# tsnorri/vcf2multialign

Measured on AMD Instinct MI355X. Metric: aligned A2M Gbases/sec, higher is better.
Workload: dtype u8

## Files before the change

### vcf2multialign_amd/csrc/kernels.hpp

```cpp
#pragma once

#include <hip/hip_runtime.h>
#include <stdint.h>

#ifdef V2M_CHECKED_BUILD
__device__ uint32_t v2m_lds_poison_seed;
#endif

namespace v2m {

typedef uint32_t u32;
typedef uint64_t u64;

constexpr int kWave = 64;
typedef u32 vec4u __attribute__((ext_vector_type(4)));
typedef vec4u vec4u_unaligned8 __attribute__((aligned(8)));

#ifdef V2M_CHECKED_BUILD
__device__ __forceinline__ u32 poison_hash(u32 seed, u32 wg, u32 i)
{
	u32 h = seed ^ (wg * 0x9E3779B1u) ^ (i * 0x85EBCA77u);
	h ^= h >> 15; h *= 0x2C1B3C6Du;
	h ^= h >> 12; h *= 0x297A2D39u;
	h ^= h >> 15;
// ... 808 lines not shown
	u32 const *record_offset;
	u32 const *edge_end;
};

__global__ __launch_bounds__(256) void expand_reference_set_kernel(
	char const *__restrict__ ref, u32 const *__restrict__ ref_pos, u32 const *__restrict__ aln_pos,
	u32 n_nodes, set_tile_tables st, u32 n_tiles, u64 n_chunks, uint4 *__restrict__ out, char gap)
{
	u64 const c = (u64) blockIdx.x * blockDim.x + threadIdx.x;
	if (c >= n_chunks) return;
	u32 lo = 0, hi = n_tiles;
	while (hi - lo > 1) {
		u32 const mid = lo + (hi - lo) / 2;
		if ((u64) st.record_offset[mid] <= c * 16) lo = mid; else hi = mid;
	}
	u64 const p0 = (u64) st.col_begin[lo] + (c * 16 - st.record_offset[lo]);
	out[c] = expand_reference_chunk(ref, ref_pos, aln_pos, n_nodes, st.col_end[lo], p0, gap, (unsigned char) gap);
}


struct row_segments {
	u32 const *seg_offsets;
	u32 const *seg_edge_begin;
	u32 const *seg_copy;
	u64 const *assembled;
	u32 assembled_words;
};

__device__ __forceinline__ u64 load_row_word(
	u64 const *__restrict__ paths, u64 words_per_copy, row_segments const &rs, u32 row, u32 s_begin, u32 s_end, u32 wi)
{
	if (s_end - s_begin == 1) {
		u32 const copy = rs.seg_copy[s_begin];
		return (copy == 0xFFFFFFFFu) ? 0 : paths[(u64) copy * words_per_copy + wi];
	}
	return rs.assembled[(u64) row * rs.assembled_words + wi];
}

__global__ __launch_bounds__(256) void assemble_row_bits_kernel(
	u64 const *__restrict__ paths, u64 words_per_copy, row_segments rs, u64 *__restrict__ assembled, u32 n_words, u32 row_base, u32 word_base)
{
	__shared__ unsigned long long acc[256];
	u32 const row = blockIdx.y + row_base;
	u32 const s_begin = rs.seg_offsets[row], s_end = rs.seg_offsets[row + 1];
	if (s_end - s_begin <= 1) return;
	V2M_POISON_LDS(acc);
	u32 const lane = threadIdx.x & 63, wave = threadIdx.x >> 6;
	u32 const w0 = word_base + (blockIdx.x * 4 + wave) * 64;
	acc[threadIdx.x] = 0;
	__syncthreads();
	if (w0 < n_words) {
		u64 const e_lo = (u64) w0 * 64;
		u64 const e_hi = (u64) (w0 + 64 < n_words ? w0 + 64 : n_words) * 64;
		u32 lo = s_begin, hi = s_end;
		while (hi - lo > 1) {
			u32 const mid = lo + (hi - lo) / 2;
			if (rs.seg_edge_begin[mid] <= e_lo) lo = mid; else hi = mid;
		}
		for (u32 s = lo + lane; s < s_end; s += 64) {
			u64 b = rs.seg_edge_begin[s];
			if (b >= e_hi) break;
			u64 e = (s + 1 < s_end) ? rs.seg_edge_begin[s + 1] : ~0ULL;
			u32 const copy = rs.seg_copy[s];
			if (copy == 0xFFFFFFFFu) continue;
			b = b > e_lo ? b : e_lo;
			e = e < e_hi ? e : e_hi;
			if (b >= e) continue;
			u64 const *const column = paths + (u64) copy * words_per_copy;
			for (u64 wi = b >> 6; wi <= (e - 1) >> 6; ++wi) {
				u64 const base = wi * 64;
				u32 const from = b > base ? (u32) (b - base) : 0;
				u32 const to = e < base + 64 ? (u32) (e - base) : 64;
				u64 const mask = (to >= 64 ? ~0ULL : ((1ULL << to) - 1)) & ~((1ULL << from) - 1);
				u64 const v = column[wi] & mask;
				if (v) atomicOr(&acc[wave * 64 + (u32) (wi - w0)], (unsigned long long) v);
			}
		}
	}
	__syncthreads();
	if (w0 + lane < n_words) assembled[(u64) row * rs.assembled_words + w0 + lane] = acc[threadIdx.x];
}

constexpr int kResolveWordsPerThread = 8;
constexpr u32 kResolveQueueShards = 1024;
constexpr u32 kMaxBackWords = 2048;

__device__ __forceinline__ u64 resolve_word_exact(
	u64 const *__restrict__ paths, u64 words_per_copy, row_segments const &rs, u32 row, u32 s_begin, u32 s_end,
	edge_span const *__restrict__ spans, u64 const *__restrict__ overlappable,
	u32 wi, u64 w, u64 ovl_w, u32 *__restrict__ needs_serial, u32 max_back_words)
{
	u64 const ov = w & ovl_w;
	if (0 == ov) return w;
	int const b0 = __builtin_ctzll(ov);
	u32 sw = wi;
	int sb = 0;
	u64 fixed = ~ovl_w & ((1ULL << b0) - 1);
	if (fixed) {
		sb = 63 - __builtin_clzll(fixed);
	} else {
		u32 steps = 0;
		for (;;) {
			if (0 == sw) { sb = 0; break; }
			--sw;
			if (++steps > max_back_words) { atomicOr(&needs_serial[row], 1u); return w; }
			fixed = ~overlappable[sw];
			if (fixed) { sb = 63 - __builtin_clzll(fixed); break; }
		}
	}
	u64 out = (sw == wi) ? (w & ((1ULL << sb) - 1)) : 0;
	u32 cur = 0;
	for (u32 ww = sw; ww <= wi; ++ww) {
		u64 x = (ww == wi) ? w : load_row_word(paths, words_per_copy, rs, row, s_begin, s_end, ww);
		if (ww == sw) x &= ~((1ULL << sb) - 1);
		while (x) {
			constexpr int kBatch = 8;
			edge_span sp[kBatch];
			int bit[kBatch];
			bool has[kBatch];
#pragma unroll
			for (int k = 0; k < kBatch; ++k) {
				has[k] = 0 != x;
				bit[k] = has[k] ? __builtin_ctzll(x) : 0;
				x &= x - 1;
				sp[k] = spans[ww * 64u + bit[k]];
			}
#pragma unroll
			for (int k = 0; k < kBatch; ++k) {
				if (has[k] && sp[k].src >= cur) {
					cur = sp[k].tgt;
					if (ww == wi) out |= 1ULL << bit[k];
				}
			}
		}
	}
	return out;
}

__global__ __launch_bounds__(256) void resolve_effective_edges_kernel(
	u64 const *__restrict__ paths, u64 words_per_copy, u32 n_edges,
	row_segments rs, edge_span const *__restrict__ spans, u64 const *__restrict__ overlappable,
	u32 const *__restrict__ ovl_rank, u64 const *__restrict__ blocker_masks,
	u64 *__restrict__ eff, u32 n_words, u32 eff_words_per_row, u32 row_base, u32 word_base,
	u32 *__restrict__ queue, u32 *__restrict__ queue_counts , u32 shard_capacity, u32 *__restrict__ needs_serial, u32 max_back_words)
{
	u32 const row = blockIdx.x + row_base;
	u32 const shard = (blockIdx.y * gridDim.x + blockIdx.x) % kResolveQueueShards;
	u32 const s_begin = rs.seg_offsets[row], s_end = rs.seg_offsets[row + 1];
	u64 const tail_mask = (n_edges & 63) ? (1ULL << (n_edges & 63)) - 1 : ~0ULL;
	u64 const *row_words = nullptr;
	if (s_end - s_begin == 1) {
		u32 const copy = rs.seg_copy[s_begin];
		if (copy != 0xFFFFFFFFu) row_words = paths + (u64) copy * words_per_copy;
	} else {
		row_words = rs.assembled + (u64) row * rs.assembled_words;
	}
	u32 const w_first = word_base + blockIdx.y * kResolveWordsPerThread * blockDim.x + threadIdx.x;
	u64 w_all[kResolveWordsPerThread], ovl_all[kResolveWordsPerThread], mask_a[kResolveWordsPerThread], mask_b[kResolveWordsPerThread];
	u32 rank_all[kResolveWordsPerThread];
#pragma unroll
	for (int piece = 0; piece < kResolveWordsPerThread; ++piece) {
		u32 const wi = w_first + piece * blockDim.x;
		u32 const wc = wi < n_words ? wi : n_words - 1;
		w_all[piece] = row_words ? row_words[wc] : 0;
		ovl_all[piece] = overlappable[wc];
		rank_all[piece] = ovl_rank[wc];
		if (wi == (n_edges - 1) >> 6) w_all[piece] &= tail_mask;
	}
#pragma unroll
	for (int piece = 0; piece < kResolveWordsPerThread; ++piece) {
		u64 const ov = w_all[piece] & ovl_all[piece], ov2 = ov & (ov - 1);
		auto const entry = [&](u64 m) {
			return m ? rank_all[piece] + (u32) __builtin_popcountll(ovl_all[piece] & ((1ULL << __builtin_ctzll(m)) - 1)) : 0u;
		};
		mask_a[piece] = blocker_masks[entry(ov)];
		mask_b[piece] = blocker_masks[entry(ov2)];
	}
	int const lane = threadIdx.x & 63;
#pragma unroll
	for (int piece = 0; piece < kResolveWordsPerThread; ++piece) {
		u32 const wi = w_first + piece * blockDim.x;
		bool const in_range = wi < n_words;
		u64 const w = w_all[piece], ov = w & ovl_all[piece], ov2 = ov & (ov - 1);
		bool const hard = in_range && ov && ((w & mask_a[piece]) || (ov2 && ((w & mask_b[piece]) || (ov2 & (ov2 - 1)))));
		if (in_range && !hard) eff[(u64) row * eff_words_per_row + wi] = w;
		u64 const hard_lanes = __ballot(hard);
		if (hard_lanes) {
			u32 base = 0;
			if (0 == lane) base = atomicAdd(&queue_counts[shard], (u32) __builtin_popcountll(hard_lanes));
			base = __shfl(base, 0, kWave);
			if (hard) {
				u32 const slot = base + __builtin_amdgcn_mbcnt_hi((u32) (hard_lanes >> 32), __builtin_amdgcn_mbcnt_lo((u32) hard_lanes, 0));
				if (slot < shard_capacity) queue[(u64) shard * shard_capacity + slot] = (row - row_base) * n_words + wi;
				else eff[(u64) row * eff_words_per_row + wi] = resolve_word_exact(paths, words_per_copy, rs, row, s_begin, s_end, spans, overlappable, wi, w, ovl_all[piece], needs_serial, max_back_words);
			}
		}
	}
}

__global__ __launch_bounds__(256) void resolve_queued_words_kernel(
	u64 const *__restrict__ paths, u64 words_per_copy, u32 n_edges,
	row_segments rs, edge_span const *__restrict__ spans, u64 const *__restrict__ overlappable,
	u64 *__restrict__ eff, u32 n_words, u32 eff_words_per_row, u32 row_base,
	u32 const *__restrict__ queue, u32 const *__restrict__ queue_counts, u32 shard_capacity, u32 *__restrict__ needs_serial, u32 max_back_words)
{
	u32 const shard = blockIdx.x % kResolveQueueShards, part = blockIdx.x / kResolveQueueShards, parts = gridDim.x / kResolveQueueShards;
	u32 const n = queue_counts[shard] < shard_capacity ? queue_counts[shard] : shard_capacity;
	u64 const tail_mask = (n_edges & 63) ? (1ULL << (n_edges & 63)) - 1 : ~0ULL;
	for (u32 i = part * blockDim.x + threadIdx.x; i < n; i += parts * blockDim.x) {
		u32 const entry = queue[(u64) shard * shard_capacity + i];
		u32 const row = row_base + entry / n_words, wi = entry % n_words;
		u32 const s_begin = rs.seg_offsets[row], s_end = rs.seg_offsets[row + 1];
		u64 w = load_row_word(paths, words_per_copy, rs, row, s_begin, s_end, wi);
		if (wi == (n_edges - 1) >> 6) w &= tail_mask;
		eff[(u64) row * eff_words_per_row + wi] = resolve_word_exact(paths, words_per_copy, rs, row, s_begin, s_end, spans, overlappable, wi, w, overlappable[wi], needs_serial, max_back_words);
	}
}


__global__ __launch_bounds__(256) void resolve_rows_serial_kernel(
	u64 const *__restrict__ paths, u64 words_per_copy, u32 n_edges,
	row_segments rs, edge_span const *__restrict__ spans,
	u64 *__restrict__ eff, u64 eff_words_per_row, u32 n_rows, u32 const *__restrict__ needs_serial,
	u32 word_begin , u32 word_end)
{
	int const lane = threadIdx.x & 63;
	u32 const row = blockIdx.x * (blockDim.x >> 6) + (threadIdx.x >> 6);
	if (row >= n_rows) return;
	if (needs_serial && 0 == needs_serial[row]) return;

	u32 const s_begin = rs.seg_offsets[row], s_end = rs.seg_offsets[row + 1];
	u32 const n_words = (n_edges + 63) / 64;
	u64 *const eff_row = eff + (u64) row * eff_words_per_row;
	u32 cur = 0;

	for (u32 base = word_begin; base < word_end; base += 64) {
		u32 const wi = base + lane;
		u64 w = 0;
		if (wi < word_end) {
			w = load_row_word(paths, words_per_copy, rs, row, s_begin, s_end, wi);
			if (wi == n_words - 1 && (n_edges & 63))
				w &= (1ULL << (n_edges & 63)) - 1;
		}

		u32 lane_max = 0;
		for (u64 m = w; m; m &= m - 1) {
			u32 const e = wi * 64u + __builtin_ctzll(m);
			u32 const tgt = spans[e].tgt;
			lane_max = tgt > lane_max ? tgt : lane_max;
		}
		u32 incl = lane_max;
#pragma unroll
		for (int d = 1; d < 64; d <<= 1) {
			u32 const o = __shfl_up(incl, d, kWave);
			if (lane >= d) incl = o > incl ? o : incl;
		}
		u32 excl = __shfl_up(incl, 1, kWave);
		if (lane == 0) excl = 0;
		u32 const chunk_max = __shfl(incl, 63, kWave);

		u32 run = excl > cur ? excl : cur;
		bool uncertain = false;
		for (u64 m = w; m; m &= m - 1) {
			u32 const e = wi * 64u + __builtin_ctzll(m);
			edge_span const sp = spans[e];
			uncertain |= sp.src < run;
			run = sp.tgt > run ? sp.tgt : run;
		}

		u64 out = w;
		if (__any(uncertain)) {
			out = 0;
			u32 c = cur;
			u64 busy = __ballot(w != 0);
			while (busy) {
				int const j = __builtin_ctzll(busy);
				busy &= busy - 1;
				if (lane == j) {
					for (u64 m = w; m; m &= m - 1) {
// ... 1256 lines not shown
```

### vcf2multialign_amd/csrc/v2m_hip.hip

```cpp

#include <hip/hip_runtime.h>

#include <algorithm>
#include <atomic>
#include <chrono>
#include <condition_variable>
#include <cstdarg>
#include <cstdio>
#include <cstdlib>
#include <cstring>
#include <memory>
#include <mutex>
#include <string>
#include <thread>
#include <utility>
#include <vector>

#include <type_traits>

#include "../../include/v2m_hip.h"
#include "kernels.hpp"
#include "founder_kernels.hpp"
#include "bgzf_kernels.hpp"
#include "vcf_kernels.hpp"
// ... 103 lines not shown
struct held_ring_state {
	std::mutex mutex;
	std::condition_variable released;
};

struct v2m_row_hold {
	pinned_buf host;
	hipEvent_t copied{};
	uint64_t outstanding{};
	held_ring_state *ring{};
};


struct word_range { u64 restart, lo, hi, stride; };

struct row_view {
	u64 begin{}, end{};
	u64 max_unaligned{};
	u32 n_tiles{};
	dev_buf d_template, d_template0;
	bool has_template0{};
	dev_buf d_edge_begin, d_cross_offsets, d_cross_edges;
	word_range words{};
	u64 length() const { return end - begin; }
};


struct v2m_ctx {
	int device{};
	u32 n_cus{256};
	hipStream_t stream{};
	hipStream_t copy_stream{};
	std::string err;

	bool profiling{};
	std::vector<event_pair> events[V2M_KERNEL_END];
	std::vector<event_pair> free_events;

	bool has_graph{};
	u64 n_nodes{}, n_edges{}, ref_len{}, aligned_len{}, label_bytes{};
	bool has_nul_byte{};
	std::vector<u32> h_csum;
	std::vector<u32> h_tgt_prefix_max;
	dev_buf d_ref, d_ref_pos, d_aln_pos, d_spans, d_patches, d_labels, d_overlappable;
	dev_buf d_ovl_rank, d_blocker_masks;
	std::vector<u32> h_aln_pos, h_tile_edge_begin, h_cross_offsets, h_cross_edges;
	std::vector<v2m::edge_patch> h_patches;
	std::vector<u64> h_overlappable;

	row_view whole, window;
	bool windowed{};
	row_view &view() { return set_call ? set.view : windowed ? window : whole; }
	row_view const &view() const { return set_call ? set.view : windowed ? window : whole; }

	struct window_set {
		row_view view;
		u64 n_windows{}, pitch{}, mean_tile_bytes{};
		std::vector<u32> lengths;
		dev_buf d_col_begin, d_col_end, d_record_offset, d_edge_end, d_tile_window, d_first_tile, d_slot_offset32;
	} set;
	bool has_set{}, set_call{};
	scratch_buf d_set_tile_offsets, d_set_lengths[2];
	int set_lengths_slot{};

	u64 const *d_paths{};
	dev_buf owned_paths;
	dev_buf d_slice_src;
	u64 path_rows{}, path_cols{};
	u64 path_pitch{};
	dev_buf d_by_edge;
	bool by_edge_valid{};

	struct transpose_pick { u64 rows, cols, src_pitch, dst_pitch; std::string kernel; };
	std::vector<transpose_pick> transpose_choice;

	int store_mode{-1};
	int unaligned_store_mode{-1};
	std::string info;

	pinned_buf h_row_stage[2];
	hipEvent_t ev_row_stage[2]{};
	bool row_stage_in_flight[2]{};
	int row_stage_next{};
	scratch_buf d_resolve_queue, d_resolve_count;
	scratch_buf d_eff, d_row_bits, d_seg_offsets, d_seg_edge_begin, d_seg_copy, d_sums, d_lengths, d_needs_serial, d_tile_counts, d_row_lengths;
	scratch_buf ring[2];
	dev_buf d_ops_ref_before;
	bool has_ops_ref_before{};
	scratch_buf d_ops_info, d_ops_offsets, d_ops_counts, d_ops_base, d_ops_out;
	pinned_buf h_ops_stage, h_ops_out;
	std::vector<v2m_aln_op> ops_row;
	held_ring_state held_state;
	std::vector<std::unique_ptr<v2m_row_hold>> host_slots;
	pinned_buf trials_stage[2];
	scratch_buf d_bgzf_slots, d_bgzf_sizes, d_bgzf_offsets, d_bgzf_table, d_bgzf_dense[2], d_bgzf_in;
	pinned_buf h_bgzf_table[2];
	hipEvent_t ev_compute[2]{};
	scratch_buf d_inflate_in[2], d_inflate_out[2], d_inflate_status[2];
	hipEvent_t ev_inflate_in[2]{};
	dev_buf d_vcf_text[2];
	scratch_buf d_vcf_in, d_vcf_status, d_vcf_tiles, d_vcf_tile_offsets, d_vcf_line_start, d_vcf_lines, d_vcf_gt_off, d_vcf_flags, d_vcf_tmp_begin,
		d_vcf_tmp_columns, d_vcf_totals, d_vcf_heads, d_vcf_columns, d_vcf_layout, d_vcf_wanted;
};


namespace {

int fail(v2m_ctx *ctx, int code, char const *fmt, ...)
{
	char buf[512];
	va_list ap;
	va_start(ap, fmt);
	std::vsnprintf(buf, sizeof(buf), fmt, ap);
	va_end(ap);
	if (ctx) ctx->err = buf; else g_create_error = buf;
	return code;
}

#define V2M_HIP_TRY(ctx, expr)                                                              \
	do {                                                                                    \
		hipError_t const st_ = (expr);                                                      \
		if (hipSuccess != st_) {                                                            \
			int const code_ = (hipErrorOutOfMemory == st_) ? V2M_ERR_OUT_OF_MEMORY : V2M_ERR_HIP; \
			return fail(ctx, code_, "%s failed: %s", #expr, hipGetErrorString(st_));       \
		}                                                                                   \
	} while (0)


struct timed_launch {
	v2m_ctx *ctx;
	int kernel;
	event_pair ev{};
	bool active{};

	timed_launch(v2m_ctx *c, int k) : ctx(c), kernel(k)
	{
		if (!ctx->profiling) return;
		if (!ctx->free_events.empty()) { ev = ctx->free_events.back(); ctx->free_events.pop_back(); }
		else if (hipSuccess != hipEventCreate(&ev.begin) || hipSuccess != hipEventCreate(&ev.end)) return;
		active = (hipSuccess == hipEventRecord(ev.begin, ctx->stream));
	}
	~timed_launch()
	{
		if (!active) return;
		(void) hipEventRecord(ev.end, ctx->stream);
		ctx->events[kernel].push_back(ev);
	}
};


template <typename T>
int upload_vec(v2m_ctx *ctx, dev_buf &dst, std::vector<T> const &src, size_t min_bytes = 16)
{
	size_t const bytes(std::max(src.size() * sizeof(T), min_bytes));
	V2M_HIP_TRY(ctx, dst.ensure(bytes));
	if (!src.empty())
		V2M_HIP_TRY(ctx, hipMemcpyAsync(dst.p, src.data(), src.size() * sizeof(T), hipMemcpyHostToDevice, ctx->stream));
	return V2M_OK;
}


struct scoped_events {
	std::vector<hipEvent_t> ev;
	~scoped_events() { for (auto e : ev) (void) hipEventDestroy(e); }
	hipError_t create(std::size_t n)
	{
		for (std::size_t i(0); i < n; ++i) {
			hipEvent_t e{};
// ... 234 lines not shown
	if (shape == "stream4x64") return launch_transpose_stream<4, 16, 4, 4, 64>(ctx, d_src, SW, DW, SP, DP, d_dst, xcd, order);
#endif
	if (shape == "8x8") return launch_transpose_shape<8, 8>(ctx, d_src, SW, DW, SP, DP, d_dst, xcd, order);
#ifdef V2M_TUNING_BUILD
	if (shape == "4x16") return launch_transpose_shape<4, 16>(ctx, d_src, SW, DW, SP, DP, d_dst, xcd, order);
	if (shape == "16x8") return launch_transpose_shape<16, 8>(ctx, d_src, SW, DW, SP, DP, d_dst, xcd, order);
	if (shape == "16x4") return launch_transpose_shape<16, 4>(ctx, d_src, SW, DW, SP, DP, d_dst, xcd, order);
	if (shape == "4x8") return launch_transpose_shape<4, 8>(ctx, d_src, SW, DW, SP, DP, d_dst, xcd, order);
	if (shape == "8x4") return launch_transpose_shape<8, 4>(ctx, d_src, SW, DW, SP, DP, d_dst, xcd, order);
	if (shape == "8x16") return launch_transpose_shape<8, 16>(ctx, d_src, SW, DW, SP, DP, d_dst, xcd, order);
#endif
	return fail(ctx, V2M_ERR_INVALID_ARGUMENT, "unknown transpose kernel '%s'", shape.c_str());
}

char const *const kTransposeCandidates[] = {"8x8", "stream16", "lines8", "lines16"};

int launch_transpose(v2m_ctx *ctx, u64 const *d_src, u64 n_rows, u64 n_cols, u64 *d_dst, u64 src_pitch = 0, u64 dst_pitch = 0)
{
	u64 const SW(n_rows / 64), DW(n_cols / 64);
	u64 const SP(src_pitch ? src_pitch : SW), DP(dst_pitch ? dst_pitch : DW);
	char const *e(std::getenv("V2M_TRANSPOSE_PANEL"));
	if (e && *e) return launch_transpose_named(ctx, e, d_src, SW, DW, SP, DP, d_dst);
	if (SW * DW * 512 < (u64(32) << 20)) return launch_transpose_named(ctx, "8x8", d_src, SW, DW, SP, DP, d_dst);
	for (auto const &c : ctx->transpose_choice)
		if (c.rows == n_rows && c.cols == n_cols && c.src_pitch == SP && c.dst_pitch == DP) return launch_transpose_named(ctx, c.kernel, d_src, SW, DW, SP, DP, d_dst);

	std::vector<std::string> names;
	if (char const *list = std::getenv("V2M_TRANSPOSE_CANDIDATES")) {
		std::string cur;
		for (char const *p(list); ; ++p) {
			if (';' == *p || 0 == *p) { if (!cur.empty()) names.push_back(cur); cur.clear(); if (0 == *p) break; }
			else cur.push_back(*p);
		}
	}
	if (names.empty()) names.assign(std::begin(kTransposeCandidates), std::end(kTransposeCandidates));

	std::vector<float> best(names.size(), 1e30f);
	{
		scoped_events ev;
		V2M_HIP_TRY(ctx, ev.create(names.size() + 1));
		scoped_profiling_off const quiet(ctx);
		std::vector<char> usable(names.size(), 1);
		for (int rep(0); rep < 3; ++rep) {
			V2M_HIP_TRY(ctx, hipEventRecord(ev[0], ctx->stream));
			for (std::size_t k(0); k < names.size(); ++k) {
				if (usable[k]) {
					int const rc(launch_transpose_named(ctx, names[k], d_src, SW, DW, SP, DP, d_dst));
					if (V2M_ERR_UNSUPPORTED == rc) usable[k] = 0;
					else if (rc) return rc;
				}
				V2M_HIP_TRY(ctx, hipEventRecord(ev[k + 1], ctx->stream));
			}
			V2M_HIP_TRY(ctx, hipStreamSynchronize(ctx->stream));
			for (std::size_t k(0); k < names.size(); ++k) {
				float ms(0);
				V2M_HIP_TRY(ctx, hipEventElapsedTime(&ms, ev[k], ev[k + 1]));
				if (rep && usable[k]) best[k] = std::min(best[k], ms);
			}
		}
		if (std::none_of(usable.begin(), usable.end(), [](char u) { return 0 != u; })) return fail(ctx, V2M_ERR_UNSUPPORTED, "matrix too large for one transpose launch");
		if (std::any_of(usable.begin(), usable.end(), [](char u) { return 0 == u; })) ctx->err.clear();
	}
	std::size_t const pick(std::size_t(std::min_element(best.begin(), best.end()) - best.begin()));
	ctx->transpose_choice.push_back({n_rows, n_cols, SP, DP, names[pick]});
	std::string note("transpose " + std::to_string(n_rows) + "x" + std::to_string(n_cols) + " bits" + ((SP != SW || DP != DW) ? " (column pitches " + std::to_string(SP) + " / " + std::to_string(DP) + " words)" : std::string()) + ": " + names[pick] + " (");
	for (std::size_t k(0); k < names.size(); ++k) {
		char buf[64];
		std::snprintf(buf, sizeof(buf), "%s%s %.3f ms", k ? ", " : "", names[k].c_str(), best[k]);
		note += buf;
	}
	note += ")";
	if (ctx->info.size() > 2000) ctx->info.clear();
	if (!ctx->info.empty()) ctx->info += "; ";
	ctx->info += note;
	return launch_transpose_named(ctx, names[pick], d_src, SW, DW, SP, DP, d_dst);
}


struct prepared_rows {
	u32 *seg_offsets{};
	u32 *seg_edge_begin{};
	u32 *seg_copy{};
	u64 n_rows{}, n_segments{};
	bool any_switching_row{};
};

int prepare_rows(v2m_ctx *ctx, v2m_row_batch const *rows, u64 row_begin, u64 row_end, prepared_rows &out)
{
	u64 const n_rows(row_end - row_begin);
	u64 max_segments(n_rows);
	if (rows->cut_offsets) {
		for (u64 r(row_begin); r < row_end; ++r) {
			if (rows->cut_offsets[r + 1] < rows->cut_offsets[r])
				return fail(ctx, V2M_ERR_INVALID_ARGUMENT, "cut_offsets decrease at row %llu", (unsigned long long) r);
			max_segments += rows->cut_offsets[r + 1] - rows->cut_offsets[r];
		}
	}
	if (max_segments >= 0xFFFFFFFFull)
		return fail(ctx, V2M_ERR_UNSUPPORTED, "row batch has too many cut segments (%llu) for one call", (unsigned long long) max_segments);
	auto const pad([](u64 n) { return (n * sizeof(u32) + 63) & ~u64(63); });
	int const area(ctx->row_stage_next);
	if (ctx->row_stage_in_flight[area]) {
		V2M_HIP_TRY(ctx, hipEventSynchronize(ctx->ev_row_stage[area]));
		ctx->row_stage_in_flight[area] = false;
	}
	V2M_HIP_TRY(ctx, ctx->h_row_stage[area].ensure(pad(n_rows + 1) + 2 * pad(max_segments)));
	char *const base(static_cast<char *>(ctx->h_row_stage[area].p));
	V2M_POISON_HOST(base, pad(n_rows + 1) + 2 * pad(max_segments));
	out.seg_offsets = reinterpret_cast<u32 *>(base);
	out.seg_edge_begin = reinterpret_cast<u32 *>(base + pad(n_rows + 1));
	out.seg_copy = reinterpret_cast<u32 *>(base + pad(n_rows + 1) + pad(max_segments));
	out.n_rows = n_rows;
	out.any_switching_row = false;

	out.seg_offsets[0] = 0;
	for (u64 r(row_begin); r < row_end; ++r) {
		u64 const c_begin(rows->cut_offsets ? rows->cut_offsets[r] : 0), c_end(rows->cut_offsets ? rows->cut_offsets[r + 1] : 0);
		u64 const n_seg(c_begin == c_end ? 1 : (c_end - c_begin) + (0 != rows->cut_nodes[c_begin] ? 1 : 0));
		out.seg_offsets[r - row_begin + 1] = u32(out.seg_offsets[r - row_begin] + n_seg);
		out.any_switching_row = out.any_switching_row || n_seg > 1;
	}
	out.n_segments = out.seg_offsets[n_rows];

	struct row_error { int code{V2M_OK}; std::string text; };
	auto const fill_row([&](u64 r, row_error &err) {
		auto const failed([&](int code, char const *fmt, unsigned long long a, unsigned long long b = 0) {
			char buf[256];
			std::snprintf(buf, sizeof(buf), fmt, a, b);
			err.code = code;
			err.text = buf;
		});
		u64 const c_begin(rows->cut_offsets ? rows->cut_offsets[r] : 0), c_end(rows->cut_offsets ? rows->cut_offsets[r + 1] : 0);
		u32 n(out.seg_offsets[r - row_begin]);
		if (c_begin == c_end) {
			if (!rows->copy_index) return failed(V2M_ERR_INVALID_ARGUMENT, "row %llu has no cuts and rows->copy_index is NULL", r);
			u32 const copy(rows->copy_index[r]);
			if (copy != V2M_PLOIDY_MAX && (!ctx->d_paths || copy >= ctx->path_cols))
				return failed(V2M_ERR_INVALID_ARGUMENT, "row %llu: chromosome copy %llu is outside the path matrix", r, copy);
			out.seg_edge_begin[n] = 0;
			out.seg_copy[n] = copy;
			return;
		}
		u64 prev(0);
		for (u64 k(c_begin); k < c_end; ++k) {
			u64 const node(rows->cut_nodes[k]);
			u32 const copy(rows->cut_copies[k]);
			if (node >= ctx->n_nodes) return failed(V2M_ERR_PRECONDITION, "row %llu: cut node %llu does not exist", r, node);
			if (k > c_begin && node <= prev) return failed(V2M_ERR_PRECONDITION, "row %llu: cut nodes must be strictly increasing", r);
			if (copy != V2M_PLOIDY_MAX && (!ctx->d_paths || copy >= ctx->path_cols))
				return failed(V2M_ERR_INVALID_ARGUMENT, "row %llu: chromosome copy %llu is outside the path matrix", r, copy);
			u32 const first_edge(ctx->h_csum[node]);
			if (node > 0 && ctx->h_tgt_prefix_max[first_edge] > node)
				return failed(V2M_ERR_PRECONDITION, "row %llu: cut node %llu lies inside the span of an ALT edge", r, node);
			if (k == c_begin && node != 0) {
				out.seg_edge_begin[n] = 0;
				out.seg_copy[n] = V2M_PLOIDY_MAX;
				++n;
			}
			out.seg_edge_begin[n] = first_edge;
			out.seg_copy[n] = copy;
			++n;
			prev = node;
		}
	});
	std::vector<row_error> errors(n_rows);
	unsigned const n_threads(out.n_segments >= (u64(1) << 20) ? unsigned(std::min<u64>(n_rows, 8)) : 1u);
	if (n_threads <= 1) {
		for (u64 r(row_begin); r < row_end; ++r) { fill_row(r, errors[r - row_begin]); if (V2M_OK != errors[r - row_begin].code) break; }
	}
	else {
		std::atomic<u64> next(row_begin);
		auto const work([&] { for (u64 r; (r = next.fetch_add(1)) < row_end;) fill_row(r, errors[r - row_begin]); });
		std::vector<std::thread> pool;
		for (unsigned t(1); t < n_threads; ++t) pool.emplace_back(work);
		work();
		for (auto &t : pool) t.join();
	}
	for (auto const &e : errors) if (V2M_OK != e.code) return fail(ctx, e.code, "%s", e.text.c_str());
	return V2M_OK;
}


int forced_store_mode(bool unaligned)
{
	if (unaligned) {
		char const *const e = std::getenv("V2M_UNALIGNED_STORE");
		if (e && 0 == std::strcmp(e, "plain")) return 0;
		if (e && 0 == std::strcmp(e, "nt")) return 1;
		return -1;
	}
	char const *e = std::getenv("V2M_NT_STORES");
	if (!(e && *e)) return -1;
	return std::atoi(e) != 0 ? 1 : 0;
}

u32 rows_per_group_for(u64 n_rows)
{
	char const *e = std::getenv("V2M_ROWS_PER_GROUP");
	int const v((e && *e) ? std::atoi(e) : 0);
	if (v > 0) return u32(std::min(v, 256));
	return u32(std::min<u64>(32, std::max<u64>(1, n_rows)));
}


u32 rows_per_group_for_set(u64 n_rows, u64 mean_tile_bytes)
{
	char const *e = std::getenv("V2M_ROWS_PER_GROUP");
	if (e && *e && std::atoi(e) > 0) return rows_per_group_for(n_rows);
	u64 const by_bytes(32 * u64(v2m::kTileBytes) / std::max<u64>(1, mean_tile_bytes));
	return u32(std::min<u64>(std::max<u64>(1, n_rows), std::min<u64>(256, std::max<u64>(32, by_bytes))));
}


int expand_reference(v2m_ctx *ctx, row_view const &v, dev_buf &dst, char gap)
{
	u64 const n_chunks(u64(v.n_tiles) * v2m::kTileChunks);
	V2M_HIP_TRY(ctx, dst.ensure(n_chunks * 16));
	{
		timed_launch tl(ctx, V2M_KERNEL_TEMPLATE);
		hipLaunchKernelGGL(v2m::expand_reference_row_kernel, dim3(unsigned((n_chunks + 255) / 256)), dim3(256), 0, ctx->stream,
			ctx->d_ref.as<char>(), ctx->d_ref_pos.as<u32>(), ctx->d_aln_pos.as<u32>(), u32(ctx->n_nodes), u32(v.end), n_chunks, dst.as<uint4>(), gap, u32(v.begin));
	}
	V2M_HIP_TRY(ctx, hipGetLastError());
	return V2M_OK;
}


int resolve_slice(v2m_ctx *ctx, v2m_row_batch const *rows, u64 row_begin, u64 row_end)
{
	u64 const n_rows(row_end - row_begin);
	word_range const wr(ctx->view().words);
	u64 const eff_words(wr.stride), n_words(wr.hi);
	if (0 == ctx->n_edges) return V2M_OK;

	prepared_rows pr;
	if (int const rc = prepare_rows(ctx, rows, row_begin, row_end, pr)) return rc;
	if (wr.lo >= wr.hi) return V2M_OK;
	auto const upload([&](scratch_buf &dst, u32 const *src, u64 count) -> int {
		V2M_HIP_TRY(ctx, dst.ensure(std::max<size_t>(count * sizeof(u32), 16)));
		if (count) V2M_HIP_TRY(ctx, hipMemcpyAsync(dst.p, src, count * sizeof(u32), hipMemcpyHostToDevice, ctx->stream));
		return V2M_OK;
	});
	int const stage(ctx->row_stage_next);
	ctx->row_stage_in_flight[stage] = true;
	ctx->row_stage_next ^= 1;
	int upload_rc(upload(ctx->d_seg_offsets, pr.seg_offsets, n_rows + 1));
	if (!upload_rc) upload_rc = upload(ctx->d_seg_edge_begin, pr.seg_edge_begin, pr.n_segments);
	if (!upload_rc) upload_rc = upload(ctx->d_seg_copy, pr.seg_copy, pr.n_segments);
	hipError_t const recorded(hipEventRecord(ctx->ev_row_stage[stage], ctx->stream));
	if (upload_rc) return upload_rc;
	V2M_HIP_TRY(ctx, recorded);
	V2M_HIP_TRY(ctx, ctx->d_eff.ensure(n_rows * eff_words * sizeof(u64)));
	V2M_HIP_TRY(ctx, ctx->d_needs_serial.ensure(n_rows * sizeof(u32)));
	V2M_HIP_TRY(ctx, hipMemsetAsync(ctx->d_needs_serial.p, 0, n_rows * sizeof(u32), ctx->stream));

	bool const any_switching_row(pr.any_switching_row);
	if (any_switching_row) V2M_HIP_TRY(ctx, ctx->d_row_bits.ensure(n_rows * eff_words * sizeof(u64)));

	u64 *const d_eff(ctx->d_eff.as<u64>() - wr.restart);
	u64 *const d_row_bits(any_switching_row ? ctx->d_row_bits.as<u64>() - wr.restart : nullptr);
	v2m::row_segments rs{ctx->d_seg_offsets.as<u32>(), ctx->d_seg_edge_begin.as<u32>(), ctx->d_seg_copy.as<u32>(), d_row_bits, u32(eff_words)};
	char const *const back_env(std::getenv("V2M_MAX_BACK_WORDS"));
	u32 const max_back_words((back_env && *back_env) ? u32(std::strtoul(back_env, nullptr, 10)) : v2m::kMaxBackWords);
	char const *const capacity_env(std::getenv("V2M_RESOLVE_QUEUE_CAPACITY"));
	bool const capacity_forced(capacity_env && *capacity_env);
	{
		timed_launch tl(ctx, V2M_KERNEL_RESOLVE);
		u64 const rows_per_launch(std::max<u64>(1, std::min<u64>(65535, 0xFFFFFFFFull / std::max<u64>(1, n_words))));
		u64 const assembled_words(n_words - wr.restart), resolved_words(n_words - wr.lo);
		for (u64 r0(0); r0 < n_rows; r0 += rows_per_launch) {
			u64 const nr(std::min<u64>(rows_per_launch, n_rows - r0));
			if (any_switching_row)
				for (u64 y0(0); y0 < nr; y0 += 65535)
					hipLaunchKernelGGL(v2m::assemble_row_bits_kernel, dim3(unsigned((assembled_words + 255) / 256), unsigned(std::min<u64>(65535, nr - y0))), dim3(256), 0, ctx->stream,
						ctx->d_paths, ctx->path_pitch, rs, d_row_bits, u32(n_words), u32(r0 + y0), u32(wr.restart));
			u64 const shard_capacity(capacity_forced ? std::min<u64>(std::strtoull(capacity_env, nullptr, 10), (u64(1) << 28) / v2m::kResolveQueueShards)
				: std::max<u64>(256, std::min<u64>(nr * resolved_words, u64(1) << 28) / v2m::kResolveQueueShards));
			V2M_HIP_TRY(ctx, ctx->d_resolve_queue.ensure(shard_capacity * v2m::kResolveQueueShards * sizeof(u32)));
			V2M_HIP_TRY(ctx, ctx->d_resolve_count.ensure(v2m::kResolveQueueShards * sizeof(u32)));
			V2M_HIP_TRY(ctx, hipMemsetAsync(ctx->d_resolve_count.p, 0, v2m::kResolveQueueShards * sizeof(u32), ctx->stream));
			for (u64 piece0(0), pieces((resolved_words + 256 * v2m::kResolveWordsPerThread - 1) / (256 * v2m::kResolveWordsPerThread)); piece0 < pieces; piece0 += 65535)
				hipLaunchKernelGGL(v2m::resolve_effective_edges_kernel, dim3(unsigned(nr), unsigned(std::min<u64>(65535, pieces - piece0))), dim3(256), 0, ctx->stream,
					ctx->d_paths, ctx->path_pitch, u32(ctx->n_edges), rs, ctx->d_spans.as<v2m::edge_span>(), ctx->d_overlappable.as<u64>(),
					ctx->d_ovl_rank.as<u32>(), ctx->d_blocker_masks.as<u64>(),
					d_eff, u32(n_words), u32(eff_words), u32(r0), u32(wr.lo + piece0 * 256 * v2m::kResolveWordsPerThread),
					ctx->d_resolve_queue.as<u32>(), ctx->d_resolve_count.as<u32>(), u32(shard_capacity), ctx->d_needs_serial.as<u32>(), max_back_words);
			hipLaunchKernelGGL(v2m::resolve_queued_words_kernel, dim3(2 * v2m::kResolveQueueShards), dim3(256), 0, ctx->stream,
				ctx->d_paths, ctx->path_pitch, u32(ctx->n_edges), rs, ctx->d_spans.as<v2m::edge_span>(), ctx->d_overlappable.as<u64>(),
				d_eff, u32(n_words), u32(eff_words), u32(r0),
				ctx->d_resolve_queue.as<u32>(), ctx->d_resolve_count.as<u32>(), u32(shard_capacity), ctx->d_needs_serial.as<u32>(), max_back_words);
		}
		hipLaunchKernelGGL(v2m::resolve_rows_serial_kernel, dim3(unsigned((n_rows + 3) / 4)), dim3(256), 0, ctx->stream,
			ctx->d_paths, ctx->path_pitch, u32(ctx->n_edges), rs, ctx->d_spans.as<v2m::edge_span>(),
			d_eff, eff_words, u32(n_rows), ctx->d_needs_serial.as<u32>(), u32(wr.restart), u32(n_words));
	}
	V2M_HIP_TRY(ctx, hipGetLastError());
	return V2M_OK;
}


struct splice_grid {
	u32 rows_per_group, n_groups, tile_run;
	u64 n_blocks;
};

u32 tile_run_for(u32 n_tiles)
{
	char const *e = std::getenv("V2M_TILE_RUN");
	int const v((e && *e) ? std::atoi(e) : 0);
	u32 const run(v > 0 ? u32(v) : 64u);
	return std::max<u32>(1, std::min(run, n_tiles));
}

int make_grid(v2m_ctx *ctx, u64 n_rows, splice_grid &g)
{
	g.rows_per_group = ctx->set_call ? rows_per_group_for_set(n_rows, ctx->set.mean_tile_bytes) : rows_per_group_for(n_rows);
	g.n_groups = u32((n_rows + g.rows_per_group - 1) / g.rows_per_group);
	g.n_blocks = u64(ctx->view().n_tiles) * g.n_groups;
	g.tile_run = tile_run_for(ctx->view().n_tiles);
	if (g.n_blocks > 0x7FFFFFFFull)
		return fail(ctx, V2M_ERR_UNSUPPORTED, "splice grid too large (%llu workgroups); use smaller batches", (unsigned long long) g.n_blocks);
	return V2M_OK;
}


template <typename F>
int store_flavour_launch(v2m_ctx *ctx, bool unaligned, u64 n_rows, u64 bytes, F const &launch)
{
	int &slot(unaligned ? ctx->unaligned_store_mode : ctx->store_mode);
	int mode(forced_store_mode(unaligned));
	if (mode < 0) mode = slot;
	if (mode < 0 && bytes >= (u64(1) << 30)) {
		scoped_events ev;
		V2M_HIP_TRY(ctx, ev.create(5));
		V2M_HIP_TRY(ctx, hipEventRecord(ev[0], ctx->stream));
		for (int i(0); i < 4; ++i) {
			launch(0 == (i & 1));
			V2M_HIP_TRY(ctx, hipEventRecord(ev[i + 1], ctx->stream));
		}
		V2M_HIP_TRY(ctx, hipStreamSynchronize(ctx->stream));
		float t[4];
		for (int i(0); i < 4; ++i) V2M_HIP_TRY(ctx, hipEventElapsedTime(&t[i], ev[i], ev[i + 1]));
		float const nt_ms(std::min(t[0], t[2])), plain_ms(std::min(t[1], t[3]));
		slot = nt_ms <= plain_ms ? 1 : 0;
		char buf[160];
		std::snprintf(buf, sizeof(buf), "%s splice stores: %s (calibrated on %llu rows: nontemporal %.3f ms, plain %.3f ms)",
			unaligned ? "unaligned" : "aligned", slot ? "nontemporal" : "plain", (unsigned long long) n_rows, nt_ms, plain_ms);
		if (unaligned && ctx->info.size() > 2000) ctx->info.clear();
		if (!ctx->info.empty()) ctx->info += "; ";
		ctx->info += buf;
		mode = slot;
	}
	if (mode < 0) mode = 1;
	{
		timed_launch tl(ctx, unaligned ? V2M_KERNEL_SPLICE_UNALIGNED : V2M_KERNEL_SPLICE_ALIGNED);
		launch(0 != mode);
	}
	V2M_HIP_TRY(ctx, hipGetLastError());
	return V2M_OK;
}


v2m::set_tile_tables set_tables(v2m_ctx const *ctx)
{
	auto const &s(ctx->set);
	return {s.d_col_begin.as<u32>(), s.d_col_end.as<u32>(), s.d_record_offset.as<u32>(), s.d_edge_end.as<u32>()};
}

int expand_reference_set(v2m_ctx *ctx, dev_buf &dst, char gap);


int splice_aligned_slice(v2m_ctx *ctx, v2m_row_batch const *rows, u64 row_begin, u64 row_end, char *d_out, u64 row_pitch)
{
	u64 const n_rows(row_end - row_begin);
	if (0 == n_rows || 0 == ctx->aligned_len) return V2M_OK;
	if (int const rc = resolve_slice(ctx, rows, row_begin, row_end)) return rc;

// ... 2348 lines not shown
```

Before: 6839.

## Process four rows per resolve block with prefetched row loads and merged uploads

The resolve kernel now handles a group of rows per block. Per-word overlappable and rank data are loaded once and reused across rows, and row sources are broadcast with readlane. Row words are prefetched several rows ahead, and blocker-mask gathers are skipped when no lane has overlappable bits. Queue-overflow words are deferred to a tail loop. On the host, the three segment tables go up in one memcpy and the counter and needs_serial memsets are merged into one, cutting API calls per batch. The changes add register pressure and reduce grid parallelism by the group factor.

```diff
diff --git a/vcf2multialign_amd/csrc/kernels.hpp b/vcf2multialign_amd/csrc/kernels.hpp
--- a/vcf2multialign_amd/csrc/kernels.hpp
+++ b/vcf2multialign_amd/csrc/kernels.hpp
@@ -914,6 +914,10 @@
 }
 
 constexpr int kResolveWordsPerThread = 8;
+constexpr int kResolveWordsPerPass = 2;
+constexpr int kResolveRowsPerGroup = 4;
+constexpr int kResolvePrefetchDepth = 4;
+constexpr int kResolveRowsPerRound = 1;
 constexpr u32 kResolveQueueShards = 1024;
 constexpr u32 kMaxBackWords = 2048;
 
@@ -973,60 +977,129 @@
 	u64 const *__restrict__ paths, u64 words_per_copy, u32 n_edges,
 	row_segments rs, edge_span const *__restrict__ spans, u64 const *__restrict__ overlappable,
 	u32 const *__restrict__ ovl_rank, u64 const *__restrict__ blocker_masks,
-	u64 *__restrict__ eff, u32 n_words, u32 eff_words_per_row, u32 row_base, u32 word_base,
+	u64 *__restrict__ eff, u32 n_words, u32 eff_words_per_row, u32 row_base, u32 row_end , u32 word_base,
 	u32 *__restrict__ queue, u32 *__restrict__ queue_counts , u32 shard_capacity, u32 *__restrict__ needs_serial, u32 max_back_words)
 {
-	u32 const row = blockIdx.x + row_base;
+	constexpr int K = kResolveWordsPerThread, P = kResolveWordsPerPass, R = kResolveRowsPerGroup, D = kResolvePrefetchDepth, B = kResolveRowsPerRound;
+	static_assert(K >= P && 0 == K % P && R <= 64 && R * K <= 64 && D >= B && 0 == D % B, "a lane per row of the chunk and a bit per word of a thread; whole passes; whole groups of gathers in a round");
+	u32 const lane = threadIdx.x & 63;
 	u32 const shard = (blockIdx.y * gridDim.x + blockIdx.x) % kResolveQueueShards;
-	u32 const s_begin = rs.seg_offsets[row], s_end = rs.seg_offsets[row + 1];
+	u32 const first_row = row_base + blockIdx.x * R;
+	u32 const count = row_end - first_row < (u32) R ? row_end - first_row : (u32) R;
 	u64 const tail_mask = (n_edges & 63) ? (1ULL << (n_edges & 63)) - 1 : ~0ULL;
-	u64 const *row_words = nullptr;
-	if (s_end - s_begin == 1) {
+	u32 const last_word = (n_edges - 1) >> 6;
+
+	u64 source;
+	{
+		u32 const row = first_row + (lane < count ? lane : count - 1);
+		u32 const s_begin = rs.seg_offsets[row], s_end = rs.seg_offsets[row + 1];
 		u32 const copy = rs.seg_copy[s_begin];
-		if (copy != 0xFFFFFFFFu) row_words = paths + (u64) copy * words_per_copy;
-	} else {
-		row_words = rs.assembled + (u64) row * rs.assembled_words;
-	}
-	u32 const w_first = word_base + blockIdx.y * kResolveWordsPerThread * blockDim.x + threadIdx.x;
-	u64 w_all[kResolveWordsPerThread], ovl_all[kResolveWordsPerThread], mask_a[kResolveWordsPerThread], mask_b[kResolveWordsPerThread];
-	u32 rank_all[kResolveWordsPerThread];
-#pragma unroll
-	for (int piece = 0; piece < kResolveWordsPerThread; ++piece) {
-		u32 const wi = w_first + piece * blockDim.x;
-		u32 const wc = wi < n_words ? wi : n_words - 1;
-		w_all[piece] = row_words ? row_words[wc] : 0;
-		ovl_all[piece] = overlappable[wc];
-		rank_all[piece] = ovl_rank[wc];
-		if (wi == (n_edges - 1) >> 6) w_all[piece] &= tail_mask;
-	}
-#pragma unroll
-	for (int piece = 0; piece < kResolveWordsPerThread; ++piece) {
-		u64 const ov = w_all[piece] & ovl_all[piece], ov2 = ov & (ov - 1);
-		auto const entry = [&](u64 m) {
-			return m ? rank_all[piece] + (u32) __builtin_popcountll(ovl_all[piece] & ((1ULL << __builtin_ctzll(m)) - 1)) : 0u;
+		source = (s_end - s_begin != 1) ? (u64) (rs.assembled + (u64) row * rs.assembled_words)
+			: (copy != 0xFFFFFFFFu) ? (u64) (paths + (u64) copy * words_per_copy) : 0;
+	}
+	auto const source_of = [&](u32 j) {
+		u32 const lo = __builtin_amdgcn_readlane((u32) source, j), hi = __builtin_amdgcn_readlane((u32) (source >> 32), j);
+		return (u64) hi << 32 | lo;
+	};
+
+	u32 const w_slab = word_base + blockIdx.y * (K * 256u) + threadIdx.x;
+	u64 overflow = 0;
+	for (u32 pass = 0; pass < (u32) (K / P); ++pass) {
+		u32 const w_first = w_slab + pass * (P * 256u);
+		u32 offset[P];
+		u64 ovl[P];
+		u32 rank[P];
+#pragma unroll
+		for (int k = 0; k < P; ++k) {
+			u32 const wi = w_first + k * 256u;
+			u32 const wc = wi < n_words ? wi : n_words - 1;
+			offset[k] = wc * 8u;
+			ovl[k] = overlappable[wc];
+			rank[k] = ovl_rank[wc];
+		}
+		auto const load_row = [&](u32 j, u64 (&into)[P]) {
+			u64 const s = source_of(j < count ? j : count - 1);
+			typedef char const __attribute__((address_space(1))) *global_bytes;
+			typedef u64 const __attribute__((address_space(1))) *global_word;
+			global_bytes const from = (global_bytes) (s ? s : (u64) overlappable);
+#pragma unroll
+			for (int k = 0; k < P; ++k) into[k] = *(global_word) (from + offset[k]);
 		};
-		mask_a[piece] = blocker_masks[entry(ov)];
-		mask_b[piece] = blocker_masks[entry(ov2)];
-	}
-	int const lane = threadIdx.x & 63;
-#pragma unroll
-	for (int piece = 0; piece < kResolveWordsPerThread; ++piece) {
-		u32 const wi = w_first + piece * blockDim.x;
-		bool const in_range = wi < n_words;
-		u64 const w = w_all[piece], ov = w & ovl_all[piece], ov2 = ov & (ov - 1);
-		bool const hard = in_range && ov && ((w & mask_a[piece]) || (ov2 && ((w & mask_b[piece]) || (ov2 & (ov2 - 1)))));
-		if (in_range && !hard) eff[(u64) row * eff_words_per_row + wi] = w;
-		u64 const hard_lanes = __ballot(hard);
-		if (hard_lanes) {
-			u32 base = 0;
-			if (0 == lane) base = atomicAdd(&queue_counts[shard], (u32) __builtin_popcountll(hard_lanes));
-			base = __shfl(base, 0, kWave);
-			if (hard) {
-				u32 const slot = base + __builtin_amdgcn_mbcnt_hi((u32) (hard_lanes >> 32), __builtin_amdgcn_mbcnt_lo((u32) hard_lanes, 0));
-				if (slot < shard_capacity) queue[(u64) shard * shard_capacity + slot] = (row - row_base) * n_words + wi;
-				else eff[(u64) row * eff_words_per_row + wi] = resolve_word_exact(paths, words_per_copy, rs, row, s_begin, s_end, spans, overlappable, wi, w, ovl_all[piece], needs_serial, max_back_words);
-			}
-		}
+
+		for (u32 j0 = 0; j0 < count; j0 += D) {
+			u64 ahead[D][P];
+#pragma unroll
+			for (int d = 0; d < D; ++d) load_row(j0 + d, ahead[d]);
+#pragma unroll
+			for (int d0 = 0; d0 < D; d0 += B) {
+				u32 const j = j0 + d0;
+				if (d0 > 0 && j >= count) goto pass_done;
+				u64 w[B][P], mask_a[B][P], mask_b[B][P];
+				u64 any = 0;
+#pragma unroll
+				for (int b = 0; b < B; ++b) {
+					bool const is_ref = 0 == source_of(j + b < count ? j + b : count - 1);
+#pragma unroll
+					for (int k = 0; k < P; ++k) {
+						u64 x = is_ref ? 0 : ahead[d0 + b][k];
+						if (w_first + k * 256u == last_word) x &= tail_mask;
+						w[b][k] = x;
+						any |= x & ovl[k];
+						mask_a[b][k] = mask_b[b][k] = 0;
+					}
+				}
+				if (__ballot(0 != any)) {
+#pragma unroll
+					for (int b = 0; b < B; ++b) {
+#pragma unroll
+						for (int k = 0; k < P; ++k) {
+							u64 const ov = w[b][k] & ovl[k], ov2 = ov & (ov - 1);
+							auto const entry = [&](u64 m) {
+								return m ? rank[k] + (u32) __builtin_popcountll(ovl[k] & ((1ULL << __builtin_ctzll(m)) - 1)) : 0u;
+							};
+							mask_a[b][k] = blocker_masks[entry(ov)];
+							mask_b[b][k] = blocker_masks[entry(ov2)];
+						}
+					}
+				}
+#pragma unroll
+				for (int b = 0; b < B; ++b) {
+					if (j + b >= count) break;
+					u32 const row = first_row + j + b;
+					u64 *const eff_row = eff + (u64) row * eff_words_per_row;
+#pragma unroll
+					for (int k = 0; k < P; ++k) {
+						u32 const wi = w_first + k * 256u;
+						bool const in_range = wi < n_words;
+						u64 const x = w[b][k], ov = x & ovl[k], ov2 = ov & (ov - 1);
+						bool const hard = in_range && ov && ((x & mask_a[b][k]) || (ov2 && ((x & mask_b[b][k]) || (ov2 & (ov2 - 1)))));
+						if (in_range && !hard) eff_row[wi] = x;
+						u64 const hard_lanes = __ballot(hard);
+						if (hard_lanes) {
+							u32 base = 0;
+							if (0 == lane) base = atomicAdd(&queue_counts[shard], (u32) __builtin_popcountll(hard_lanes));
+							base = __shfl(base, 0, kWave);
+							if (hard) {
+								u32 const slot = base + __builtin_amdgcn_mbcnt_hi((u32) (hard_lanes >> 32), __builtin_amdgcn_mbcnt_lo((u32) hard_lanes, 0));
+								if (slot < shard_capacity) queue[(u64) shard * shard_capacity + slot] = (row - row_base) * n_words + wi;
+								else overflow |= 1ULL << ((j + b) * K + pass * P + k);
+							}
+						}
+					}
+				}
+			}
+		}
+	pass_done:;
+	}
+
+	while (overflow) {
+		u32 const i = (u32) __builtin_ctzll(overflow);
+		overflow &= overflow - 1;
+		u32 const row = first_row + i / K, wi = w_slab + (i % K) * 256u;
+		u32 const s_begin = rs.seg_offsets[row], s_end = rs.seg_offsets[row + 1];
+		u64 x = load_row_word(paths, words_per_copy, rs, row, s_begin, s_end, wi);
+		if (wi == last_word) x &= tail_mask;
+		eff[(u64) row * eff_words_per_row + wi] = resolve_word_exact(paths, words_per_copy, rs, row, s_begin, s_end, spans, overlappable, wi, x, overlappable[wi], needs_serial, max_back_words);
 	}
 }
 
diff --git a/vcf2multialign_amd/csrc/v2m_hip.hip b/vcf2multialign_amd/csrc/v2m_hip.hip
--- a/vcf2multialign_amd/csrc/v2m_hip.hip
+++ b/vcf2multialign_amd/csrc/v2m_hip.hip
@@ -209,8 +209,10 @@
 	hipEvent_t ev_row_stage[2]{};
 	bool row_stage_in_flight[2]{};
 	int row_stage_next{};
-	scratch_buf d_resolve_queue, d_resolve_count;
-	scratch_buf d_eff, d_row_bits, d_seg_offsets, d_seg_edge_begin, d_seg_copy, d_sums, d_lengths, d_needs_serial, d_tile_counts, d_row_lengths;
+	scratch_buf d_resolve_queue;
+	scratch_buf d_resolve_flags;
+	scratch_buf d_row_tables;
+	scratch_buf d_eff, d_row_bits, d_sums, d_lengths, d_tile_counts, d_row_lengths;
 	scratch_buf ring[2];
 	dev_buf d_ops_ref_before;
 	bool has_ops_ref_before{};
@@ -611,6 +613,7 @@
 	u32 *seg_edge_begin{};
 	u32 *seg_copy{};
 	u64 n_rows{}, n_segments{};
+	size_t table_bytes{};
 	bool any_switching_row{};
 };
 
@@ -650,6 +653,7 @@
 		out.any_switching_row = out.any_switching_row || n_seg > 1;
 	}
 	out.n_segments = out.seg_offsets[n_rows];
+	out.table_bytes = size_t(pad(n_rows + 1) + pad(max_segments) + out.n_segments * sizeof(u32));
 
 	struct row_error { int code{V2M_OK}; std::string text; };
 	auto const fill_row([&](u64 r, row_error &err) {
@@ -765,30 +769,31 @@
 	prepared_rows pr;
 	if (int const rc = prepare_rows(ctx, rows, row_begin, row_end, pr)) return rc;
 	if (wr.lo >= wr.hi) return V2M_OK;
-	auto const upload([&](scratch_buf &dst, u32 const *src, u64 count) -> int {
-		V2M_HIP_TRY(ctx, dst.ensure(std::max<size_t>(count * sizeof(u32), 16)));
-		if (count) V2M_HIP_TRY(ctx, hipMemcpyAsync(dst.p, src, count * sizeof(u32), hipMemcpyHostToDevice, ctx->stream));
+	auto const upload([&]() -> int {
+		V2M_HIP_TRY(ctx, ctx->d_row_tables.ensure(pr.table_bytes));
+		V2M_HIP_TRY(ctx, hipMemcpyAsync(ctx->d_row_tables.p, pr.seg_offsets, pr.table_bytes, hipMemcpyHostToDevice, ctx->stream));
 		return V2M_OK;
 	});
 	int const stage(ctx->row_stage_next);
 	ctx->row_stage_in_flight[stage] = true;
 	ctx->row_stage_next ^= 1;
-	int upload_rc(upload(ctx->d_seg_offsets, pr.seg_offsets, n_rows + 1));
-	if (!upload_rc) upload_rc = upload(ctx->d_seg_edge_begin, pr.seg_edge_begin, pr.n_segments);
-	if (!upload_rc) upload_rc = upload(ctx->d_seg_copy, pr.seg_copy, pr.n_segments);
+	int const upload_rc(upload());
 	hipError_t const recorded(hipEventRecord(ctx->ev_row_stage[stage], ctx->stream));
 	if (upload_rc) return upload_rc;
 	V2M_HIP_TRY(ctx, recorded);
 	V2M_HIP_TRY(ctx, ctx->d_eff.ensure(n_rows * eff_words * sizeof(u64)));
-	V2M_HIP_TRY(ctx, ctx->d_needs_serial.ensure(n_rows * sizeof(u32)));
-	V2M_HIP_TRY(ctx, hipMemsetAsync(ctx->d_needs_serial.p, 0, n_rows * sizeof(u32), ctx->stream));
+	size_t const counter_bytes(v2m::kResolveQueueShards * sizeof(u32));
+	V2M_HIP_TRY(ctx, ctx->d_resolve_flags.ensure(counter_bytes + n_rows * sizeof(u32)));
+	u32 *const d_queue_counts(ctx->d_resolve_flags.as<u32>()), *const d_needs_serial(d_queue_counts + v2m::kResolveQueueShards);
 
 	bool const any_switching_row(pr.any_switching_row);
 	if (any_switching_row) V2M_HIP_TRY(ctx, ctx->d_row_bits.ensure(n_rows * eff_words * sizeof(u64)));
 
 	u64 *const d_eff(ctx->d_eff.as<u64>() - wr.restart);
 	u64 *const d_row_bits(any_switching_row ? ctx->d_row_bits.as<u64>() - wr.restart : nullptr);
-	v2m::row_segments rs{ctx->d_seg_offsets.as<u32>(), ctx->d_seg_edge_begin.as<u32>(), ctx->d_seg_copy.as<u32>(), d_row_bits, u32(eff_words)};
+	char const *const d_tables(ctx->d_row_tables.as<char>());
+	v2m::row_segments rs{reinterpret_cast<u32 const *>(d_tables), reinterpret_cast<u32 const *>(d_tables + (reinterpret_cast<char const *>(pr.seg_edge_begin) - reinterpret_cast<char const *>(pr.seg_offsets))),
+		reinterpret_cast<u32 const *>(d_tables + (reinterpret_cast<char const *>(pr.seg_copy) - reinterpret_cast<char const *>(pr.seg_offsets))), d_row_bits, u32(eff_words)};
 	char const *const back_env(std::getenv("V2M_MAX_BACK_WORDS"));
 	u32 const max_back_words((back_env && *back_env) ? u32(std::strtoul(back_env, nullptr, 10)) : v2m::kMaxBackWords);
 	char const *const capacity_env(std::getenv("V2M_RESOLVE_QUEUE_CAPACITY"));
@@ -806,22 +811,21 @@
 			u64 const shard_capacity(capacity_forced ? std::min<u64>(std::strtoull(capacity_env, nullptr, 10), (u64(1) << 28) / v2m::kResolveQueueShards)
 				: std::max<u64>(256, std::min<u64>(nr * resolved_words, u64(1) << 28) / v2m::kResolveQueueShards));
 			V2M_HIP_TRY(ctx, ctx->d_resolve_queue.ensure(shard_capacity * v2m::kResolveQueueShards * sizeof(u32)));
-			V2M_HIP_TRY(ctx, ctx->d_resolve_count.ensure(v2m::kResolveQueueShards * sizeof(u32)));
-			V2M_HIP_TRY(ctx, hipMemsetAsync(ctx->d_resolve_count.p, 0, v2m::kResolveQueueShards * sizeof(u32), ctx->stream));
+			V2M_HIP_TRY(ctx, hipMemsetAsync(d_queue_counts, 0, counter_bytes + (0 == r0 ? n_rows * sizeof(u32) : 0), ctx->stream));
 			for (u64 piece0(0), pieces((resolved_words + 256 * v2m::kResolveWordsPerThread - 1) / (256 * v2m::kResolveWordsPerThread)); piece0 < pieces; piece0 += 65535)
-				hipLaunchKernelGGL(v2m::resolve_effective_edges_kernel, dim3(unsigned(nr), unsigned(std::min<u64>(65535, pieces - piece0))), dim3(256), 0, ctx->stream,
+				hipLaunchKernelGGL(v2m::resolve_effective_edges_kernel, dim3(unsigned((nr + v2m::kResolveRowsPerGroup - 1) / v2m::kResolveRowsPerGroup), unsigned(std::min<u64>(65535, pieces - piece0))), dim3(256), 0, ctx->stream,
 					ctx->d_paths, ctx->path_pitch, u32(ctx->n_edges), rs, ctx->d_spans.as<v2m::edge_span>(), ctx->d_overlappable.as<u64>(),
 					ctx->d_ovl_rank.as<u32>(), ctx->d_blocker_masks.as<u64>(),
-					d_eff, u32(n_words), u32(eff_words), u32(r0), u32(wr.lo + piece0 * 256 * v2m::kResolveWordsPerThread),
-					ctx->d_resolve_queue.as<u32>(), ctx->d_resolve_count.as<u32>(), u32(shard_capacity), ctx->d_needs_serial.as<u32>(), max_back_words);
+					d_eff, u32(n_words), u32(eff_words), u32(r0), u32(r0 + nr), u32(wr.lo + piece0 * 256 * v2m::kResolveWordsPerThread),
+					ctx->d_resolve_queue.as<u32>(), d_queue_counts, u32(shard_capacity), d_needs_serial, max_back_words);
 			hipLaunchKernelGGL(v2m::resolve_queued_words_kernel, dim3(2 * v2m::kResolveQueueShards), dim3(256), 0, ctx->stream,
 				ctx->d_paths, ctx->path_pitch, u32(ctx->n_edges), rs, ctx->d_spans.as<v2m::edge_span>(), ctx->d_overlappable.as<u64>(),
 				d_eff, u32(n_words), u32(eff_words), u32(r0),
-				ctx->d_resolve_queue.as<u32>(), ctx->d_resolve_count.as<u32>(), u32(shard_capacity), ctx->d_needs_serial.as<u32>(), max_back_words);
+				ctx->d_resolve_queue.as<u32>(), d_queue_counts, u32(shard_capacity), d_needs_serial, max_back_words);
 		}
 		hipLaunchKernelGGL(v2m::resolve_rows_serial_kernel, dim3(unsigned((n_rows + 3) / 4)), dim3(256), 0, ctx->stream,
 			ctx->d_paths, ctx->path_pitch, u32(ctx->n_edges), rs, ctx->d_spans.as<v2m::edge_span>(),
-			d_eff, eff_words, u32(n_rows), ctx->d_needs_serial.as<u32>(), u32(wr.restart), u32(n_words));
+			d_eff, eff_words, u32(n_rows), d_needs_serial, u32(wr.restart), u32(n_words));
 	}
 	V2M_HIP_TRY(ctx, hipGetLastError());
 	return V2M_OK;
```

After: 6844 (median of 2 runs). About the same (+0.1%).
